# rotationalio/honu

Hardware: AMD Instinct MI355X
Metric: GiB/s + records/s device-resident encode+decode, 1M Large(~300KB) object batch (higher is better)
Workload: dtype u8

## Files before the change

### honu_amd/csrc/api.hip

```cpp
#include <stdio.h>
#include <stdlib.h>
#include <string.h>

#include "kernels.h"

using namespace honu;

struct honu_ctx {
    int device;
    uint64_t max_n;
    LaunchGeom geom;
    void *ws;
    uint64_t *counts;
    uint64_t *offs;
    uint64_t *totals;
    DecodeScratch *scratch;
    uint32_t *reg_inline;
    EncAclPos *enc_acl;
    FusedState dec;
    uint64_t lb_bytes;
    ScanState scan;
    uint32_t spec_off;
    int speculate;
    hipStream_t aux;
    hipEvent_t ev_fork, ev_join;
    int enc_fork;
    bool acl_inplace;
    bool reg_inplace;
    int guard_blocks;
    uint32_t copy_seq;
    int enc_form;
};

static LaunchGeom copy_geom(honu_ctx *ctx) {
    LaunchGeom g = ctx->geom;
    const uint32_t k = __atomic_fetch_add(&ctx->copy_seq, 1u, __ATOMIC_RELAXED) % COPY_TICKET_LINES;
    g.copy_tickets = ctx->geom.copy_tickets + (uint64_t)k * COPY_TICKET_STRIDE;
    return g;
}
static constexpr uint32_t SPEC_BACKOFF_CALLS = 16;
#ifndef SPECULATE_DEFAULT
#define SPECULATE_DEFAULT 2
#endif

static thread_local char g_last_error[256];

static int32_t hip_fail(hipError_t e, const char *what) {
    snprintf(g_last_error, sizeof g_last_error, "%s: %s", what, hipGetErrorString(e));
    return HONU_E_HIP;
}
#define HIPCHK(x)                                  \
    do {                                           \
        hipError_t e_ = (x);                       \
        if (e_ != hipSuccess) return hip_fail(e_, #x); \
    } while (0)

static int32_t arg_fail(const char *what) {
    snprintf(g_last_error, sizeof g_last_error, "invalid argument: %s", what);
    return HONU_E_ARG;
}

static bool aligned(const void *p, uintptr_t a) { return ((uintptr_t)p & (a - 1)) == 0; }

#define FUSED_DECODE_MIN_RECORDS (48ull << 10)

static int fused_blocks(const LaunchGeom &g) {
    const int resident = 2 * g.num_cu;
    return g.lane_blocks > 0 && g.lane_blocks < resident ? g.lane_blocks : resident;
}

template <class T>
static uint64_t carve(T *&p, void *base, uint64_t at, uint64_t count) {
    p = (T *)((uintptr_t)base + at);
    return at + count * sizeof(T);
}

static uint64_t ctx_carve(honu_ctx *c, void *base) {
    const uint64_t n = c->max_n;
    const uint64_t tiles = (n + HONU_WAVE - 1) / HONU_WAVE;
    const uint64_t groups = (tiles / HONU_WAVE + 1) > LB_GROUPS ? tiles / HONU_WAVE + 1 : LB_GROUPS;
    uint64_t at = 0;
    at = carve(c->counts, base, at, 3 * n);
    at = carve(c->offs, base, at, 3 * n);
    at = carve(c->totals, base, at, 4);
    at = carve(c->scratch, base, at, n);
    at = carve(c->reg_inline, base, at, 8 * n);
    at = carve(c->enc_acl, base, at, n);
    at = carve(c->dec.lb, base, at, 1);
    at = carve(c->scan.lb, base, at, 1);
    at = carve(c->dec.status, base, at, 3 * tiles);
    at = carve(c->dec.gstatus, base, at, 3 * groups);
    c->dec.words = 3 * tiles + 3 * groups;
    c->scan.words = scan_status_words(n);
    at = carve(c->scan.status, base, at, c->scan.words);
    return carve(c->geom.copy_tickets, base, at, (uint64_t)COPY_TICKET_LINES * COPY_TICKET_STRIDE);
}

static bool stream_is_restricted(hipStream_t s, int num_cu) {
    int prio = 0;
    if (hipStreamGetPriority(s, &prio) == hipSuccess && prio != 0) return true;
    uint32_t mask[32] = {0};
    const uint32_t words = (uint32_t)((num_cu + 31) / 32);
    if (words > 32 || hipExtStreamGetCUMask(s, words, mask) != hipSuccess) return false;
    bool any = false, all = true;
    for (int i = 0; i < num_cu; i++) {
        const bool on = mask[i / 32] >> (i % 32) & 1u;
        any |= on;
        all &= on;
    }
    return any && !all;
}

static int env_int(const char *name, int dflt) {
#ifdef HONU_AB
    const char *v = getenv(name);
    return v && *v ? atoi(v) : dflt;
#else
    (void)name;
    return dflt;
#endif
}

extern "C" {

uint32_t honu_abi_version(void) { return HONU_ABI_VERSION; }
uint64_t honu_sizeof_meta(void) { return sizeof(honu_meta); }
uint64_t honu_sizeof_acl(void) { return sizeof(honu_acl); }
uint64_t honu_sizeof_collection(void) { return sizeof(honu_collection); }
uint64_t honu_sizeof_index(void) { return sizeof(honu_index); }
uint64_t honu_sizeof_record_info(void) { return sizeof(honu_record_info); }
uint64_t honu_sizeof_seek(void) { return sizeof(honu_seek); }
uint64_t honu_sizeof_list_row(void) { return sizeof(honu_list_row); }
uint64_t honu_sizeof_next(void) { return sizeof(honu_next); }
const char *honu_last_error(void) { return g_last_error; }

const char *honu_status_string(int32_t st) {
    switch (st) {
    case HONU_OK: return "ok";
    case HONU_ERR_BAD_VERSION: return "object is malformed: cannot decode specified version";
    case HONU_ERR_MALFORMED: return "object is malformed: cannot parse data or metadata";
    case HONU_ERR_EOF: return "EOF";
    case HONU_ERR_UNEXPECTED_EOF: return "unexpected EOF";
    case HONU_ERR_NO_LENGTH: return "field not written with length value";
    case HONU_ERR_PARSE_BOOLEAN: return "could not parse boolean value";
    case HONU_ERR_PARSE_VARINT: return "could not parse varint";
    case HONU_ERR_PANIC: return "input on which the Go reference panics";
    case HONU_ERR_CAPACITY: return "output capacity exceeded";
    case HONU_ERR_INPUT: return "input span or list outside its arena";
    case HONU_UNPARSED: return "metadata not decoded (headers only)";
    case HONU_E_ARG: return "invalid argument";
    case HONU_E_WORKSPACE: return "batch larger than the context's reserved records";
    case HONU_E_HIP: return "HIP runtime error";
    case HONU_E_NO_DEVICE: return "no gfx950 device";
    default: return "unknown status";
    }
}

honu_ctx *honu_ctx_create(int device, uint64_t max_records, int32_t *err) {
    int32_t dummy;
    if (!err) err = &dummy;
    *err = HONU_OK;
    int count = 0;
    if (hipGetDeviceCount(&count) != hipSuccess || device < 0 || device >= count) {
        snprintf(g_last_error, sizeof g_last_error, "no HIP device %d (count %d)", device, count);
        *err = HONU_E_NO_DEVICE;
        return nullptr;
    }
    hipDeviceProp_t prop;
    if (hipGetDeviceProperties(&prop, device) != hipSuccess ||
        strncmp(prop.gcnArchName, "gfx950", 6) != 0) {
        snprintf(g_last_error, sizeof g_last_error, "device %d is %s, this build targets gfx950",
                 device, prop.gcnArchName);
        *err = HONU_E_NO_DEVICE;
        return nullptr;
    }
    if (hipSetDevice(device) != hipSuccess) {
        *err = HONU_E_HIP;
        return nullptr;
    }
    honu_ctx *c = (honu_ctx *)calloc(1, sizeof(honu_ctx));
    if (!c) {
        *err = HONU_E_HIP;
        return nullptr;
    }
    auto fail = [&](int32_t e, const char *what) -> honu_ctx * {
        if (what) snprintf(g_last_error, sizeof g_last_error, "%s", what);
        if (c->ev_join) (void)hipEventDestroy(c->ev_join);
        if (c->ev_fork) (void)hipEventDestroy(c->ev_fork);
        if (c->aux) (void)hipStreamDestroy(c->aux);
        if (c->dec.spec_seen) (void)hipHostFree(c->dec.spec_seen);
        if (c->ws) (void)hipFree(c->ws);
        free(c);
        *err = e;
        return nullptr;
    };
    c->device = device;
    c->max_n = max_records ? max_records : 1;
    c->geom.num_cu = prop.multiProcessorCount;
    c->geom.per_record_blocks = env_int("HONU_RECORD_BLOCKS", prop.multiProcessorCount * 8);
    c->geom.lane_blocks = env_int("HONU_LANE_BLOCKS", 0);
    c->geom.copy_blocks = env_int("HONU_COPY_BLOCKS", prop.multiProcessorCount * 2);
    c->geom.record_variant = env_int("HONU_RECORD_VARIANT", 0);
    if (c->geom.record_variant != 5 && c->geom.record_variant != 6)
        c->geom.record_variant = 0;
    c->acl_inplace = env_int("HONU_ACL_INPLACE", 1) != 0;
    c->reg_inplace = env_int("HONU_REGIONS_INPLACE", 1) != 0;
    c->guard_blocks = env_int("HONU_GUARD_BLOCKS", 0);
    if (c->guard_blocks < 0) c->guard_blocks = 0;
    const uint64_t end = ctx_carve(c, nullptr), bytes = end + 256;
    if (hipMalloc(&c->ws, bytes) != hipSuccess) {
        c->ws = nullptr;
        char msg[96];
        snprintf(msg, sizeof msg, "hipMalloc(%llu) failed", (unsigned long long)bytes);
        return fail(HONU_E_HIP, msg);
    }
    if (hipHostMalloc((void **)&c->dec.spec_seen, 2 * sizeof(uint32_t),
                      hipHostMallocMapped | hipHostMallocCoherent) != hipSuccess) {
        c->dec.spec_seen = nullptr;
        return fail(HONU_E_HIP, "hipHostMalloc(spec_seen) failed");
    }
    c->dec.spec_seen[0] = 0;
    c->dec.spec_seen[1] = 0;
    c->speculate = SPECULATE_DEFAULT;
    c->enc_fork = env_int("HONU_ENCODE_FORK", 2);
    if (c->enc_fork < 0 || c->enc_fork > 2) c->enc_fork = 2;
    if (hipStreamCreateWithFlags(&c->aux, hipStreamNonBlocking) != hipSuccess) {
        c->aux = nullptr;
        return fail(HONU_E_HIP, "stream creation failed");
    }
    if (hipEventCreateWithFlags(&c->ev_fork, hipEventDisableTiming) != hipSuccess) {
        c->ev_fork = nullptr;
        return fail(HONU_E_HIP, "event creation failed");
    }
    if (hipEventCreateWithFlags(&c->ev_join, hipEventDisableTiming) != hipSuccess) {
        c->ev_join = nullptr;
        return fail(HONU_E_HIP, "event creation failed");
    }
    ctx_carve(c, c->ws);
    c->lb_bytes = (uint64_t)((uint8_t *)c->ws + end - (uint8_t *)c->dec.lb);
    c->geom.copy_steal = 1;
    c->scan.max_blocks = 4 * prop.multiProcessorCount;
    hipStream_t s = nullptr;
    bool ok = hipStreamCreateWithFlags(&s, hipStreamNonBlocking) == hipSuccess;
    ok = ok && hipMemsetAsync(c->dec.lb, 0, c->lb_bytes, s) == hipSuccess;
    ok = ok && hipStreamSynchronize(s) == hipSuccess;
    if (s) (void)hipStreamDestroy(s);
    if (!ok) return fail(HONU_E_HIP, "look-back state initialisation failed");
    return c;
}

int32_t honu_ctx_reset(honu_ctx *ctx, void *stream) {
    if (!ctx) return arg_fail("ctx");
    HIPCHK(hipSetDevice(ctx->device));
    HIPCHK(hipMemsetAsync(ctx->dec.lb, 0, ctx->lb_bytes, (hipStream_t)stream));
    HIPCHK(hipStreamSynchronize((hipStream_t)stream));
    return HONU_OK;
}

void honu_ctx_destroy(honu_ctx *ctx) {
    if (!ctx) return;
    (void)hipSetDevice(ctx->device);
    (void)hipStreamSynchronize(ctx->aux);
    (void)hipEventDestroy(ctx->ev_fork);
    (void)hipEventDestroy(ctx->ev_join);
    (void)hipStreamDestroy(ctx->aux);
    (void)hipFree(ctx->ws);
    (void)hipHostFree(ctx->dec.spec_seen);
    free(ctx);
}

uint64_t honu_ctx_max_records(const honu_ctx *ctx) { return ctx ? ctx->max_n : 0; }

int32_t honu_ctx_set_param(honu_ctx *ctx, const char *name, int64_t value) {
    if (!ctx || !name) return arg_fail("ctx/name");
    if (!strcmp(name, "copy_blocks") && value > 0) ctx->geom.copy_blocks = (int)value;
    else if (!strcmp(name, "record_blocks") && value > 0) ctx->geom.per_record_blocks = (int)value;
    else if (!strcmp(name, "lane_blocks") && value >= 0) ctx->geom.lane_blocks = (int)value;
    else if (!strcmp(name, "speculate") && value >= 0 && value <= 2) ctx->speculate = (int)value;
    else if (!strcmp(name, "encode_fork") && value >= 0 && value <= 2) ctx->enc_fork = (int)value;
    else if (!strcmp(name, "acl_inplace") && (value == 0 || value == 1)) ctx->acl_inplace = value != 0;
    else if (!strcmp(name, "regions_inplace") && (value == 0 || value == 1)) ctx->reg_inplace = value != 0;
    else if (!strcmp(name, "guard_blocks") && value >= 0 && value <= 65536) ctx->guard_blocks = (int)value;
    else if (!strcmp(name, "speculate_backoff") && value >= 0 && value <= (int64_t)SPEC_BACKOFF_CALLS) {
        __atomic_store_n(ctx->dec.spec_seen, 0u, __ATOMIC_RELAXED);
        ctx->spec_off = (uint32_t)value;
    }
    else if (!strcmp(name, "copy_steal") && (value == 0 || value == 1)) ctx->geom.copy_steal = (int)value;
    else if (!strcmp(name, "copy_variant") || !strcmp(name, "encode_variant") || !strcmp(name, "inline_recovery")) {
        if (value != 0) return arg_fail(name);
    }
    else if (!strcmp(name, "record_variant") &&
             (value == 0 || value == 5 || value == 6))
        ctx->geom.record_variant = (int)value;
    else if (!strcmp(name, "seek_variant") && value >= 0 && value <= 2) ctx->geom.seek_variant = (int)value;
    else return arg_fail(name);
    return HONU_OK;
}

int32_t honu_ctx_get_param(const honu_ctx *ctx, const char *name, int64_t *value) {
    if (!ctx || !name || !value) return arg_fail("ctx/name/value");
    if (!strcmp(name, "copy_blocks")) *value = ctx->geom.copy_blocks;
    else if (!strcmp(name, "record_blocks")) *value = ctx->geom.per_record_blocks;
    else if (!strcmp(name, "lane_blocks")) *value = ctx->geom.lane_blocks;
    else if (!strcmp(name, "speculate")) *value = ctx->speculate;
    else if (!strcmp(name, "encode_fork")) *value = ctx->enc_fork;
    else if (!strcmp(name, "acl_inplace")) *value = ctx->acl_inplace ? 1 : 0;
    else if (!strcmp(name, "regions_inplace")) *value = ctx->reg_inplace ? 1 : 0;
    else if (!strcmp(name, "guard_blocks")) *value = ctx->guard_blocks;
    else if (!strcmp(name, "recoveries"))
        *value = __atomic_load_n(ctx->dec.spec_seen + 1, __ATOMIC_RELAXED);
    else if (!strcmp(name, "speculate_backoff"))
        *value = __atomic_load_n(ctx->dec.spec_seen, __ATOMIC_RELAXED) ? SPEC_BACKOFF_CALLS : ctx->spec_off;
    else if (!strcmp(name, "copy_steal")) *value = ctx->geom.copy_steal;
    else if (!strcmp(name, "copy_variant") || !strcmp(name, "encode_variant") || !strcmp(name, "inline_recovery"))
        *value = 0;
    else if (!strcmp(name, "record_variant")) *value = ctx->geom.record_variant;
    else if (!strcmp(name, "walk_flag_checks")) *value = decode_walk_flag_checks();
    else if (!strcmp(name, "sort_tile")) *value = sort_tile();
    else if (!strcmp(name, "seek_variant")) *value = ctx->geom.seek_variant;
    else if (!strcmp(name, "seek_fence")) *value = seek_fence();
    else if (!strcmp(name, "seek_auto_probes")) *value = (int64_t)seek_auto_probes();
    else if (!strcmp(name, "seek_auto_keys")) *value = (int64_t)seek_auto_keys();
    else if (!strcmp(name, "merge_tile")) *value = merge_tile();
    else if (!strcmp(name, "delete_tile")) *value = delete_tile();
    else if (!strcmp(name, "list_tile")) *value = list_tile();
    else if (!strcmp(name, "list_stage")) *value = list_stage();
    else if (!strcmp(name, "filter_tile")) *value = filter_tile();
    else if (!strcmp(name, "compare_tile")) *value = compare_tile();
    else if (!strcmp(name, "compare_stage")) *value = compare_stage();
    else if (!strcmp(name, "reclaim_tile")) *value = reclaim_tile();
    else return arg_fail(name);
    return HONU_OK;
}

int32_t honu_encode_sizes(honu_ctx *ctx, const honu_meta *d_meta, uint64_t var_len,
                          const honu_acl *d_acl, uint64_t acl_len, const uint32_t *d_regions,
                          uint64_t regions_len, const uint64_t *d_payload_off, uint64_t n,
                          uint64_t *d_sizes, int32_t *d_status, void *stream) {
    if (!ctx) return arg_fail("ctx");
    if (n && (!d_meta || !d_payload_off || !d_sizes)) return arg_fail("null pointer");
    if (!aligned(d_meta, 16)) return arg_fail("rows must be 16-byte aligned");
    if (!aligned(d_acl, 4) || !aligned(d_regions, 4)) return arg_fail("tables must be 4-byte aligned");
    HIPCHK(hipSetDevice(ctx->device));
    HIPCHK(launch_encode_sizes_grp(d_meta, var_len, d_acl, acl_len, d_regions, regions_len,
                                   d_payload_off, n, d_sizes, d_status, ctx->geom.lane_blocks,
                                   (hipStream_t)stream));
    return HONU_OK;
}

int32_t honu_exclusive_scan(honu_ctx *ctx, const uint64_t *d_in, uint64_t n, uint64_t *d_out,
                            void *stream) {
    if (!ctx) return arg_fail("ctx");
    if (n > ctx->max_n) return HONU_E_WORKSPACE;
    HIPCHK(hipSetDevice(ctx->device));
    HIPCHK(launch_scan(d_in, n, 1, d_out, d_out + n, ctx->scan, (hipStream_t)stream));
    return HONU_OK;
}

static int32_t encode_records(honu_ctx *ctx, const honu_meta *d_meta, const uint8_t *d_var,
                              const honu_acl *d_acl, const uint32_t *d_regions, const uint8_t *units,
                              const uint64_t *d_payload_off, uint64_t n, uint8_t *d_out,
                              uint64_t out_cap, const uint64_t *d_out_off, int32_t *d_status,
                              void *stream) {
    if (!ctx) return arg_fail("ctx");
    if (n && (!d_meta || !d_payload_off || !d_out || !d_out_off || !d_status))
        return arg_fail("null pointer");
    if (!aligned(d_out, 16) || !aligned(d_meta, 16))
        return arg_fail("records arena and rows must be 16-byte aligned");
    if (!aligned(d_acl, 4) || !aligned(d_regions, 4)) return arg_fail("tables must be 4-byte aligned");
    HIPCHK(hipSetDevice(ctx->device));
    if (n > ctx->max_n) return HONU_E_WORKSPACE;
    ctx->enc_form = units ? 2 : 1;
    hipStream_t s = (hipStream_t)stream;
    const bool fork = ctx->enc_fork == 1 ||
                      (ctx->enc_fork == 2 && ctx->geom.lane_blocks > 0 && n &&
                       !stream_is_restricted(s, ctx->geom.num_cu));
    if (fork && n) {
        HIPCHK(hipEventRecord(ctx->ev_fork, s));
        HIPCHK(hipStreamWaitEvent(ctx->aux, ctx->ev_fork, 0));
        HIPCHK(launch_encode_acl_grp_self(d_meta, d_acl, d_payload_off, n, d_out, out_cap, d_out_off, d_status,
                                          ctx->geom.lane_blocks, ctx->aux));
        HIPCHK(hipEventRecord(ctx->ev_join, ctx->aux));
        HIPCHK(launch_encode_meta_lane(d_meta, d_var, d_acl, d_regions, d_payload_off, n, d_out,
                                       out_cap, d_out_off, d_status, ctx->enc_acl,
                                       ctx->geom.lane_blocks, ctx->geom.num_cu, units, s));
        HIPCHK(hipStreamWaitEvent(s, ctx->ev_join, 0));
        return HONU_OK;
    }
    HIPCHK(launch_encode_meta_lane(d_meta, d_var, d_acl, d_regions, d_payload_off, n, d_out,
                                   out_cap, d_out_off, d_status, ctx->enc_acl,
                                   ctx->geom.lane_blocks, ctx->geom.num_cu, units, s));
    HIPCHK(launch_encode_acl_grp(d_meta, d_acl, n, d_out, d_status, ctx->enc_acl,
                                 ctx->geom.lane_blocks, s));
    return HONU_OK;
}

int32_t honu_encode_records(honu_ctx *ctx, const honu_meta *d_meta, const uint8_t *d_var,
                            const honu_acl *d_acl, const uint32_t *d_regions,
                            const uint64_t *d_payload_off, uint64_t n, uint8_t *d_out,
                            uint64_t out_cap, const uint64_t *d_out_off, int32_t *d_status,
                            void *stream) {
    return encode_records(ctx, d_meta, d_var, d_acl, d_regions, nullptr, d_payload_off, n, d_out, out_cap,
                          d_out_off, d_status, stream);
}

int32_t honu_encode_records_units(honu_ctx *ctx, const honu_meta *d_meta, const uint8_t *d_var,
                                  const honu_acl *d_acl, const uint32_t *d_regions,
                                  const uint8_t *d_payload, const uint64_t *d_payload_off, uint64_t n,
                                  uint8_t *d_out, uint64_t out_cap, const uint64_t *d_out_off,
                                  int32_t *d_status, void *stream) {
    if (n && !d_payload) return arg_fail("null pointer");
    return encode_records(ctx, d_meta, d_var, d_acl, d_regions, d_payload, d_payload_off, n, d_out, out_cap,
                          d_out_off, d_status, stream);
}

static int32_t encode_payloads(honu_ctx *ctx, const uint8_t *d_payload, const uint64_t *d_payload_off,
                               uint64_t n, uint8_t *d_out, uint64_t out_cap, const uint64_t *d_out_off,
                               const int32_t *d_status, bool units, void *stream) {
    if (!ctx) return arg_fail("ctx");
    if (n && (!d_payload_off || !d_out || !d_out_off || !d_status)) return arg_fail("null pointer");
    if (!aligned(d_out, 16)) return arg_fail("records arena must be 16-byte aligned");
    if (ctx->enc_form && ctx->enc_form != (units ? 2 : 1))
        return arg_fail(units ? "honu_encode_payloads_units after honu_encode_records (mixed forms)"
                              : "honu_encode_payloads after honu_encode_records_units (mixed forms)");
    HIPCHK(hipSetDevice(ctx->device));
    HIPCHK(launch_encode_copy(copy_geom(ctx), d_payload, d_payload_off, n, d_out, out_cap, d_out_off,
                              d_status, units, (hipStream_t)stream));
    return HONU_OK;
}

int32_t honu_encode_payloads(honu_ctx *ctx, const uint8_t *d_payload, const uint64_t *d_payload_off,
                             uint64_t n, uint8_t *d_out, uint64_t out_cap, const uint64_t *d_out_off,
                             const int32_t *d_status, void *stream) {
    return encode_payloads(ctx, d_payload, d_payload_off, n, d_out, out_cap, d_out_off, d_status, false, stream);
}

int32_t honu_encode_payloads_units(honu_ctx *ctx, const uint8_t *d_payload, const uint64_t *d_payload_off,
                                   uint64_t n, uint8_t *d_out, uint64_t out_cap, const uint64_t *d_out_off,
                                   const int32_t *d_status, void *stream) {
    return encode_payloads(ctx, d_payload, d_payload_off, n, d_out, out_cap, d_out_off, d_status, true, stream);
}

int32_t honu_encode(honu_ctx *ctx, const honu_meta *d_meta, const uint8_t *d_var, uint64_t var_len,
                    const honu_acl *d_acl, uint64_t acl_len, const uint32_t *d_regions,
                    uint64_t regions_len, const uint8_t *d_payload, const uint64_t *d_payload_off,
                    uint64_t n, uint8_t *d_out, uint64_t out_cap, const uint64_t *d_out_off,
                    int32_t *d_status, void *stream) {
    (void)var_len;
    (void)acl_len;
    (void)regions_len;
    if (!d_payload) {
        int32_t st = honu_encode_records(ctx, d_meta, d_var, d_acl, d_regions, d_payload_off, n, d_out,
                                         out_cap, d_out_off, d_status, stream);
        if (st) return st;
        return honu_encode_payloads(ctx, d_payload, d_payload_off, n, d_out, out_cap, d_out_off, d_status,
                                    stream);
    }
    int32_t st = honu_encode_records_units(ctx, d_meta, d_var, d_acl, d_regions, d_payload, d_payload_off, n,
                                           d_out, out_cap, d_out_off, d_status, stream);
    if (st) return st;
    return honu_encode_payloads_units(ctx, d_payload, d_payload_off, n, d_out, out_cap, d_out_off,
                                      d_status, stream);
}

int32_t honu_marshal_batch(honu_ctx *ctx, const honu_meta *d_meta, const uint8_t *d_var,
                           uint64_t var_len, const honu_acl *d_acl, uint64_t acl_len,
// ... 644 lines not shown
```

### honu_amd/csrc/copy.hip

```cpp
#include "kernels.h"

namespace honu {

struct EncodeSegments {
    const uint8_t *payload;
    const uint64_t *payload_off;
    uint8_t *out;
    uint64_t out_cap;
    const uint64_t *out_off;
    const int32_t *status;

    HONU_DEV uint64_t start(uint64_t i) const { return payload_off[i]; }
    HONU_DEV uint64_t lo() const { return payload_off[0]; }
    bool units;
    HONU_DEV bool get(uint64_t i, uint64_t &len, const uint8_t *&src, uint8_t *&dst, uint64_t &skip) const {
        const int32_t st = status[i];
        const uint64_t o0 = out_off[i], o1 = out_off[i + 1];
        const uint64_t s = payload_off[i];
        len = payload_off[i + 1] - s;
        src = payload + s;
        dst = out + o0 + 1 + uvarint_len(len);
        skip = 0;
        if (units) {
            const uint64_t a0 = (uint64_t)dst, a1 = a0 + len;
            const uint64_t h_end = ((a0 + PAYLOAD_UNIT - 1) & ~(PAYLOAD_UNIT - 1)) < a1
                                       ? ((a0 + PAYLOAD_UNIT - 1) & ~(PAYLOAD_UNIT - 1)) : a1;
            const uint64_t t_beg = (a1 & ~(PAYLOAD_UNIT - 1)) > h_end ? (a1 & ~(PAYLOAD_UNIT - 1)) : h_end;
            skip = h_end - a0;
            len = t_beg - h_end;
            src += skip;
            dst += skip;
        }
        return st == HONU_OK && o1 <= out_cap && len != 0;
    }
};

struct DecodeSegments {
    const uint8_t *rec;
    const honu_record_info *info;
    const DecodeScratch *scratch;
    const uint64_t *offs;
    uint8_t *data;

    HONU_DEV uint64_t start(uint64_t i) const { return offs[3 * i + 2]; }
    HONU_DEV uint64_t lo() const { return 0; }
    uint64_t n_;
    HONU_DEV bool get(uint64_t i, uint64_t &len, const uint8_t *&src, uint8_t *&dst, uint64_t &skip) const {
        skip = 0;
        const int32_t st = info[i].data_status;
        len = info[i].data_len;
        src = rec + scratch[i].data_src;
        dst = data + offs[3 * i + 2];
        return st == HONU_OK && len != 0;
    }
};

struct SpanSegments {
    const uint8_t *rec;
    const honu_record_info *info;
    const DecodeScratch *scratch;
    const uint64_t *offs;
    uint8_t *data;

    HONU_DEV uint64_t start(uint64_t i) const { return offs[i]; }
    HONU_DEV uint64_t lo() const { return 0; }
    HONU_DEV bool get(uint64_t i, uint64_t &len, const uint8_t *&src, uint8_t *&dst, uint64_t &skip) const {
        skip = 0;
        const int32_t st = info[i].data_status;
        len = info[i].data_len;
        src = rec + scratch[i].data_src;
        dst = data + offs[i];
        return st == HONU_OK && len != 0;
    }
};

struct FetchSegments {
    const honu_list_row *rows;
    const uint8_t *rec;
    const uint64_t *rec_off;
    const uint64_t *val_off;
    uint8_t *values;
    uint64_t val_cap;

    HONU_DEV uint64_t start(uint64_t g) const { return val_off[g]; }
    HONU_DEV uint64_t lo() const { return 0; }
    HONU_DEV bool get(uint64_t g, uint64_t &len, const uint8_t *&src, uint8_t *&dst, uint64_t &skip) const {
        skip = 0;
        const uint64_t o0 = val_off[g], o1 = val_off[g + 1];
        const uint32_t r = rows[g].record;
        len = o1 - o0;
        const bool ok = len != 0 && o1 <= val_cap;
        src = rec + (ok ? rec_off[r] : 0);
        dst = values + o0;
        return ok;
    }
};

struct ReclaimSegments {
    const uint32_t *source;
    const uint8_t *rec;
    const uint64_t *rec_off;
    const uint64_t *val_off;
    uint8_t *values;
    uint64_t val_cap;

    HONU_DEV uint64_t start(uint64_t j) const { return val_off[j]; }
    HONU_DEV uint64_t lo() const { return 0; }
    HONU_DEV bool get(uint64_t j, uint64_t &len, const uint8_t *&src, uint8_t *&dst, uint64_t &skip) const {
        skip = 0;
        const uint64_t o0 = val_off[j], o1 = val_off[j + 1];
        const uint32_t r = source[j];
        len = o1 - o0;
        const bool ok = len != 0 && o1 <= val_cap;
        src = rec + (ok ? rec_off[r] : 0);
        dst = values + o0;
        return ok;
    }
};

#define SMALL_SEG_WAVES_FACTOR 4
#ifndef COPY_FEW_WAVES_MIN
#define COPY_FEW_WAVES_MIN (64u << 10)
#endif
constexpr int COPY_UNROLL = 4;

template <class Seg>
HONU_DEV void copy_short_run(const Seg &seg, uint64_t i0, uint64_t i1, uint64_t short_max) {
    uint64_t len_nx = 0, skip = 0;
    const uint8_t *src_nx = nullptr;
    uint8_t *dst_nx = nullptr;
    bool ok_nx = i0 < i1 && seg.get(i0, len_nx, src_nx, dst_nx, skip);
    for (uint64_t i = i0; i < i1; i++) {
        const uint64_t len = len_nx;
        const uint8_t *src = src_nx;
        uint8_t *dst = dst_nx;
        const bool ok = ok_nx;
        if (i + 1 < i1) ok_nx = seg.get(i + 1, len_nx, src_nx, dst_nx, skip);
        if (ok && len < short_max) wave_copy<COPY_UNROLL>(dst, src, len);
    }
}

template <class Seg>
HONU_DEV void copy_range(const Seg &seg, uint64_t n, uint64_t lo, uint64_t hi, bool skip_short,
                         uint64_t short_max) {
    if (lo >= hi) return;
    uint64_t a = 0, b = n;
    while (b - a > 1) {
        const uint64_t mid = (a + b) >> 1;
        if (seg.start(mid) <= lo) a = mid;
        else b = mid;
    }
    uint64_t s_nx = seg.start(a), len_nx = 0, skip_nx = 0;
    const uint8_t *src_nx = nullptr;
    uint8_t *dst_nx = nullptr;
    bool ok_nx = seg.get(a, len_nx, src_nx, dst_nx, skip_nx);
    for (uint64_t i = a; i < n; i++) {
        const uint64_t s0 = s_nx, len = len_nx, s = s0 + skip_nx;
        const uint8_t *src = src_nx;
        uint8_t *dst = dst_nx;
        const bool ok = ok_nx;
        if (s0 >= hi) break;
        if (i + 1 < n) {
            s_nx = seg.start(i + 1);
            ok_nx = seg.get(i + 1, len_nx, src_nx, dst_nx, skip_nx);
        }
        if (!ok) continue;
        if (skip_short && len < short_max) continue;
        const uint64_t x = s > lo ? s : lo;
        const uint64_t e = s + len;
        const uint64_t y = e < hi ? e : hi;
        if (x < y)
            wave_copy<COPY_UNROLL>(dst + (x - s), src + (x - s), y - x);
    }
}

#define COPY_STEAL_MIN (16u << 10)
#define COPY_STEAL 8u
template <class Seg>
__global__ __launch_bounds__(HONU_BLOCK) void k_copy_segments(Seg seg, uint64_t n,
                                                               const uint64_t *__restrict__ total_p,
                                                               uint64_t short_max, uint32_t *tickets,
                                                               uint32_t steal) {
    uint64_t W = (uint64_t)gridDim.x * HONU_WAVES_PER_BLOCK;
    const uint64_t w = (uint64_t)blockIdx.x * HONU_WAVES_PER_BLOCK + wave_in_block();
    const uint64_t base = seg.lo();
    const uint64_t total = *total_p - base;
    const bool few = n && total / n >= COPY_FEW_WAVES_MIN;
    if (few) {
        const uint64_t Wall = W;
        W /= SMALL_SEG_WAVES_FACTOR;
        if (w >= W) {
            const uint64_t v = w - W, V = Wall - W;
            copy_short_run(seg, n * v / V, n * (v + 1) / V, short_max);
            return;
        }
    }
    if (w >= W) return;
    auto range = [&](uint64_t v, uint64_t &lo, uint64_t &hi) {
        lo = base + ((total * v / W) & ~15ull);
        hi = (v + 1 == W) ? base + total : base + ((total * (v + 1) / W) & ~15ull);
    };
    uint64_t lo, hi;
    range(w, lo, hi);
    if (tickets && n && total / n >= COPY_STEAL_MIN) {
        auto cut = [&](uint64_t l, uint64_t h) {
            return h - ((((h - l) * steal) >> 6) & ~15ull);
        };
        copy_range(seg, n, lo, cut(lo, hi), few, short_max);
        for (;;) {
            uint32_t t = 0;
            if (__lane_id() == 0) t = atomicAdd(&tickets[0], 1u);
            t = __shfl(t, 0);
            if (t >= W) break;
            uint64_t l, h;
            range(t, l, h);
            copy_range(seg, n, cut(l, h), h, few, short_max);
        }
        if (__lane_id() == 0 && atomicAdd(&tickets[1], 1u) == (uint32_t)W - 1) {
            atomicExch(&tickets[0], 0u);
            atomicExch(&tickets[1], 0u);
        }
        return;
    }
    copy_range(seg, n, lo, hi, few, short_max);
}

template <class Seg>
static hipError_t launch_copy(const LaunchGeom &g, const Seg &seg, uint64_t n,
                              const uint64_t *total, uint32_t *tickets, hipStream_t s) {
    const dim3 grid(g.copy_blocks * SMALL_SEG_WAVES_FACTOR), block(HONU_BLOCK);
    hipLaunchKernelGGL((k_copy_segments<Seg>), grid, block, 0, s, seg, n, total,
                       (uint64_t)COPY_FEW_WAVES_MIN, g.copy_steal ? tickets : nullptr, COPY_STEAL);
    return hipGetLastError();
}

hipError_t launch_encode_copy(const LaunchGeom &g, const uint8_t *payload,
                              const uint64_t *payload_off, uint64_t n, uint8_t *out,
                              uint64_t out_cap, const uint64_t *out_off, const int32_t *status,
                              bool units, hipStream_t s) {
    if (n == 0) return hipSuccess;
    EncodeSegments seg{payload, payload_off, out, out_cap, out_off, status, units};
    return launch_copy(g, seg, n, payload_off + n, g.copy_tickets, s);
}

hipError_t launch_span_copy(const LaunchGeom &g, const uint8_t *rec, uint64_t n,
                            const honu_record_info *info, const DecodeScratch *scratch,
                            const uint64_t *offs, uint8_t *data, hipStream_t s) {
    if (n == 0) return hipSuccess;
    SpanSegments seg{rec, info, scratch, offs, data};
    return launch_copy(g, seg, n, offs + n, g.copy_tickets, s);
}

hipError_t launch_decode_copy(const LaunchGeom &g, const uint8_t *rec, uint64_t n,
                              const honu_record_info *info, const DecodeScratch *scratch,
                              const uint64_t *offs, const uint64_t *totals, uint8_t *data,
                              hipStream_t s) {
    if (n == 0) return hipSuccess;
    DecodeSegments seg{rec, info, scratch, offs, data, n};
    return launch_copy(g, seg, n, totals + 2, g.copy_tickets, s);
}

hipError_t launch_fetch_copy(const LaunchGeom &g, const honu_list_row *rows, uint64_t n, const uint8_t *rec,
                             const uint64_t *rec_off, const uint64_t *val_off, uint8_t *values,
                             uint64_t val_cap, hipStream_t s) {
    if (n == 0) return hipSuccess;
    FetchSegments seg{rows, rec, rec_off, val_off, values, val_cap};
    return launch_copy(g, seg, n, val_off + n, g.copy_tickets, s);
}

hipError_t launch_reclaim_copy(const LaunchGeom &g, const uint32_t *source, uint64_t n, const uint8_t *rec,
                               const uint64_t *rec_off, const uint64_t *val_off, uint8_t *values,
                               uint64_t val_cap, hipStream_t s) {
    if (n == 0) return hipSuccess;
    ReclaimSegments seg{source, rec, rec_off, val_off, values, val_cap};
    return launch_copy(g, seg, n, val_off + n, g.copy_tickets, s);
}

}
```

### honu_amd/csrc/kernels.h

```cpp
#pragma once

#include "common.h"
#include "lookback.h"

namespace honu {

struct DecodeScratch {
    uint64_t acl_pos;
    uint64_t regions_pos;
    uint64_t data_src;
    uint64_t rec_end;
};

#define GRP_ACL_FAST (1ull << 63)
#define GRP_REG_INLINE (1ull << 62)
#define GRP_ACL_A0_SHIFT 56
#define GRP_ACL_A0(pos) (((pos) >> GRP_ACL_A0_SHIFT) & 15ull)
#define GRP_ACL_TL_SHIFT 53
#define GRP_ACL_TL(pos) (((pos) >> GRP_ACL_TL_SHIFT) & 7ull)
#define GRP_POS_MASK ((1ull << GRP_ACL_TL_SHIFT) - 1)
#define ACL_ALL_PRESENT (1ull << 63)
#define PAYLOAD_UNIT 64ull

HONU_DEV void acl_enc_words(const honu_acl *e, uint32_t d[5]) {
    const uint32_t *w = reinterpret_cast<const uint32_t *>(e);
    const uint32_t e0 = w[0], e1 = w[1], e2 = w[2], e3 = w[3], e4 = w[4];
    d[0] = 1u | (e0 << 8);
    d[1] = (e0 >> 24) | (e1 << 8);
    d[2] = (e1 >> 24) | (e2 << 8);
    d[3] = (e2 >> 24) | (e3 << 8);
    d[4] = (e3 >> 24) | ((e4 & 0xFF) << 8);
}

HONU_DEV u32x4 acl_chunk(const honu_acl *A, uint64_t na, uint64_t P, uint64_t X) {
    const uint64_t j0 = (X - P) / 18;
    uint32_t b[10];
    acl_enc_words(A + j0, b);
    b[5] = b[6] = b[7] = b[8] = b[9] = 0;
    if (j0 + 1 < na) {
        uint32_t d[5];
        acl_enc_words(A + j0 + 1, d);
        b[4] = (b[4] & 0xFFFF) | (d[0] << 16);
        b[5] = (d[0] >> 16) | (d[1] << 16);
        b[6] = (d[1] >> 16) | (d[2] << 16);
        b[7] = (d[2] >> 16) | (d[3] << 16);
        b[8] = (d[3] >> 16) | (d[4] << 16);
    }
    const uint32_t off = (uint32_t)(X - (P + 18 * j0));
    const uint32_t q = off >> 2, sh = off & 3;
    uint32_t o[4];
#pragma unroll
    for (int k = 0; k < 4; k++) {
        uint32_t w0 = b[k], w1 = b[k + 1];
#pragma unroll
        for (int t = 1; t <= 4; t++)
            if ((uint32_t)t == q) {
                w0 = b[t + k];
                w1 = b[t + k + 1];
            }
        o[k] = __builtin_amdgcn_alignbyte(w1, w0, sh);
    }
    return u32x4{o[0], o[1], o[2], o[3]};
}

struct LaunchGeom {
    int num_cu;
    int per_record_blocks;
    int lane_blocks;
    int copy_blocks;
    int record_variant;
    int seek_variant;
    uint32_t *copy_tickets;
    int copy_steal;
};
#define COPY_TICKET_STRIDE 32u
#define COPY_TICKET_LINES 64u

hipError_t launch_encode_copy(const LaunchGeom &g, const uint8_t *payload,
                              const uint64_t *payload_off, uint64_t n, uint8_t *out,
                              uint64_t out_cap, const uint64_t *out_off, const int32_t *status,
                              bool units, hipStream_t s);

hipError_t launch_decode_copy(const LaunchGeom &g, const uint8_t *rec, uint64_t n,
                              const honu_record_info *info, const DecodeScratch *scratch,
                              const uint64_t *offs, const uint64_t *totals, uint8_t *data,
                              hipStream_t s);
hipError_t launch_decode_keys(const LaunchGeom &g, const honu_meta *meta,
                              const honu_record_info *info, uint64_t n, uint8_t *keys,
                              int32_t *key_status, hipStream_t s);

struct EncAclPos {
    uint64_t pos;
    uint64_t acl_off;
    uint64_t acl_count;
    uint64_t carried;
};
#define ENC_ACL_SIZED (1ull << 63)

hipError_t launch_encode_meta_lane(const honu_meta *meta, const uint8_t *var, const honu_acl *acl,
                                   const uint32_t *reg, const uint64_t *payload_off, uint64_t n,
                                   uint8_t *out, uint64_t out_cap, const uint64_t *out_off,
                                   int32_t *status, EncAclPos *acl_out, int max_blocks, int num_cu,
                                   const uint8_t *payload, hipStream_t s);
hipError_t launch_encode_acl_grp(const honu_meta *meta, const honu_acl *acl, uint64_t n,
                                 uint8_t *out, int32_t *status, const EncAclPos *acl_pos,
                                 int max_blocks, hipStream_t s);
hipError_t launch_encode_acl_grp_self(const honu_meta *meta, const honu_acl *acl, const uint64_t *payload_off,
                                      uint64_t n, uint8_t *out, uint64_t out_cap, const uint64_t *out_off,
                                      int32_t *status, int max_blocks, hipStream_t s);

hipError_t launch_encode_sizes_grp(const honu_meta *meta, uint64_t var_len, const honu_acl *acl,
                                   uint64_t acl_len, const uint32_t *reg, uint64_t reg_len,
                                   const uint64_t *payload_off, uint64_t n, uint64_t *sizes,
                                   int32_t *status, int max_blocks, hipStream_t s);
hipError_t launch_decode_fill_grp(const uint8_t *rec, uint64_t n, honu_meta *meta,
                                  honu_record_info *info, const DecodeScratch *scratch,
                                  const uint32_t *reg_inline, const uint64_t *counts,
                                  const uint64_t *offs, honu_acl *acl, uint64_t acl_cap,
                                  uint32_t *reg, uint64_t reg_cap, uint8_t *data,
                                  uint64_t data_cap, int max_blocks, hipStream_t s);

int decode_walk_flag_checks();
struct DecodeOut {
    honu_meta *meta;
    honu_record_info *info;
    honu_acl *acl;
    uint64_t acl_cap;
    uint32_t *reg;
    uint64_t reg_cap;
    uint64_t data_cap;
    int materialize;
    DecodeScratch *scratch;
    uint64_t *offs;
    uint64_t *totals;
    bool reg_inplace;
};
struct FusedState {
    LbState *lb;
    uint64_t *status, *gstatus;
    uint64_t words;
    uint32_t *spec_seen;
};
struct FusedOpts {
    int max_blocks;
    int guard_blocks;
    bool speculate;
    bool acl_inplace;
};
hipError_t launch_decode_fused(const uint8_t *rec, const uint64_t *rec_off, uint64_t n,
                               const DecodeOut &O, const FusedState &F, const FusedOpts &opt, hipStream_t s);

hipError_t launch_decode_parse_win(const uint8_t *rec, const uint64_t *rec_off, uint64_t n,
                                   honu_meta *meta, honu_record_info *info,
                                   DecodeScratch *scratch, uint32_t *reg_inline, uint64_t *counts,
                                   int max_blocks, bool inplace, bool reg_inplace, hipStream_t s);

hipError_t launch_system_sizes(const honu_collection *rows, uint64_t var_len, const honu_acl *acl,
                               uint64_t acl_len, const uint32_t *reg, uint64_t reg_len,
                               const honu_index *idx, uint64_t idx_len, uint64_t n,
                               uint64_t *sizes, int32_t *status, hipStream_t s);
hipError_t launch_system_encode(const honu_collection *rows, const uint8_t *var,
                                const honu_acl *acl, const uint32_t *reg, const honu_index *idx,
                                uint64_t n, uint8_t *out, uint64_t out_cap,
                                const uint64_t *out_off, int32_t *status, hipStream_t s);
hipError_t launch_system_parse(const uint8_t *rec, const uint64_t *rec_off, uint64_t n,
                               bool headless, honu_collection *rows, int32_t *status,
                               DecodeScratch *scratch, uint64_t *counts, hipStream_t s);
hipError_t launch_system_fill(const uint8_t *rec, uint64_t n, honu_collection *rows,
                              int32_t *status, const DecodeScratch *scratch,
                              const uint64_t *counts, const uint64_t *offs, honu_acl *acl,
                              uint64_t acl_cap, uint32_t *reg, uint64_t reg_cap, honu_index *idx,
                              uint64_t idx_cap, hipStream_t s);

hipError_t launch_decode_headers(const uint8_t *rec, const uint64_t *rec_off, uint64_t n,
                                 honu_record_info *info, hipStream_t s);
hipError_t launch_decode_spans(const uint8_t *rec, const uint64_t *rec_off, uint64_t n,
                               honu_record_info *info, DecodeScratch *scratch, uint64_t *counts,
                               hipStream_t s);
hipError_t launch_decode_data_place(uint64_t n, honu_record_info *info, const uint64_t *offs,
                                    uint64_t data_cap, hipStream_t s);
hipError_t launch_span_copy(const LaunchGeom &g, const uint8_t *rec, uint64_t n,
                            const honu_record_info *info, const DecodeScratch *scratch,
                            const uint64_t *offs, uint8_t *data, hipStream_t s);

struct ScanState {
    LbState *lb;
    uint64_t *status;
    uint64_t words;
    int max_blocks;
};
uint64_t scan_status_words(uint64_t n);
hipError_t launch_scan(const uint64_t *in, uint64_t n, int K, uint64_t *out, uint64_t *totals,
                       const ScanState &S, hipStream_t s);

inline uint64_t up256(uint64_t x) { return (x + 255) & ~255ull; }

struct SortWork {
    uint32_t *plan;
    u32x4 *key[2];
    uint32_t *idx[2];
    uint64_t *col;
    uint64_t *table;
};
uint32_t sort_tile();
uint64_t sort_workspace_bytes(uint64_t n);
SortWork sort_carve(void *work, uint64_t n);
hipError_t launch_sort_keys(const uint8_t *keys, const int32_t *status, uint64_t n, uint32_t *order,
                            uint8_t *sorted, uint64_t *valid, void *work, const ScanState &S,
                            uint64_t scan_rows, hipStream_t s);
hipError_t launch_key_objects(const uint8_t *keys, const uint32_t *order, const uint64_t *valid, uint64_t n,
                              uint64_t *obj_off, uint32_t *latest, uint64_t *objects, void *work,
                              const ScanState &S, hipStream_t s);

uint32_t seek_fence();
uint64_t seek_auto_probes();
uint64_t seek_auto_keys();
hipError_t launch_key_seek(int variant, int num_cu, const uint8_t *sorted, const uint64_t *valid, uint64_t n,
                           const uint8_t *probes, const int32_t *pstatus, uint32_t probe_len, uint64_t m,
                           const uint32_t *order, const honu_record_info *info, honu_seek *out, hipStream_t s);

uint32_t merge_tile();
hipError_t launch_key_merge(const uint8_t *sa, const uint32_t *oa, const uint64_t *valid_a, uint64_t na,
                            const uint8_t *sb, const uint32_t *ob, const uint64_t *valid_b, uint64_t nb,
                            uint32_t b_base, uint8_t *out, uint32_t *order, uint64_t *valid_out, hipStream_t s);

uint32_t delete_tile();
// ... 76 lines not shown
```

Measured before the change: 1351.

## Split copy-kernel stolen tails into geometrically shrinking pieces with a larger share

The copy kernel's work-stealing tail changes from one fixed share per wave to a configurable share split into up to four geometrically shrinking pieces, handed out through the atomic ticket counter. The share doubles when not in few-records mode. Segment lookup now uses a wave-parallel search instead of a serial binary search, and optional stage-timing stamps are added behind a compile flag. The goal is better load balance at the end of the large copy, at the cost of more atomic tickets and per-ticket index arithmetic.

```diff
diff --git a/honu_amd/csrc/api.hip b/honu_amd/csrc/api.hip
--- a/honu_amd/csrc/api.hip
+++ b/honu_amd/csrc/api.hip
@@ -38,6 +38,9 @@
     g.copy_tickets = ctx->geom.copy_tickets + (uint64_t)k * COPY_TICKET_STRIDE;
     return g;
 }
+static constexpr int COPY_TAIL_SHARE_DEFAULT = 8, COPY_TAIL_PIECES_DEFAULT = 4;
+static constexpr int64_t COPY_BLOCKS_MAX = 1 << 24;
+static_assert(16ull * COPY_BLOCKS_MAX * (COPY_PIECES_MAX + 1) < (1ull << 32), "ticket counter");
 static constexpr uint32_t SPEC_BACKOFF_CALLS = 16;
 #ifndef SPECULATE_DEFAULT
 #define SPECULATE_DEFAULT 2
@@ -200,6 +203,7 @@
     c->geom.per_record_blocks = env_int("HONU_RECORD_BLOCKS", prop.multiProcessorCount * 8);
     c->geom.lane_blocks = env_int("HONU_LANE_BLOCKS", 0);
     c->geom.copy_blocks = env_int("HONU_COPY_BLOCKS", prop.multiProcessorCount * 2);
+    if (c->geom.copy_blocks < 1 || c->geom.copy_blocks > COPY_BLOCKS_MAX) c->geom.copy_blocks = prop.multiProcessorCount * 2;
     c->geom.record_variant = env_int("HONU_RECORD_VARIANT", 0);
     if (c->geom.record_variant != 5 && c->geom.record_variant != 6)
         c->geom.record_variant = 0;
@@ -239,6 +243,8 @@
     ctx_carve(c, c->ws);
     c->lb_bytes = (uint64_t)((uint8_t *)c->ws + end - (uint8_t *)c->dec.lb);
     c->geom.copy_steal = 1;
+    c->geom.copy_tail_pieces = COPY_TAIL_PIECES_DEFAULT;
+    c->geom.copy_tail_share = COPY_TAIL_SHARE_DEFAULT;
     c->scan.max_blocks = 4 * prop.multiProcessorCount;
     hipStream_t s = nullptr;
     bool ok = hipStreamCreateWithFlags(&s, hipStreamNonBlocking) == hipSuccess;
@@ -273,7 +279,7 @@
 
 int32_t honu_ctx_set_param(honu_ctx *ctx, const char *name, int64_t value) {
     if (!ctx || !name) return arg_fail("ctx/name");
-    if (!strcmp(name, "copy_blocks") && value > 0) ctx->geom.copy_blocks = (int)value;
+    if (!strcmp(name, "copy_blocks") && value > 0 && value <= COPY_BLOCKS_MAX) ctx->geom.copy_blocks = (int)value;
     else if (!strcmp(name, "record_blocks") && value > 0) ctx->geom.per_record_blocks = (int)value;
     else if (!strcmp(name, "lane_blocks") && value >= 0) ctx->geom.lane_blocks = (int)value;
     else if (!strcmp(name, "speculate") && value >= 0 && value <= 2) ctx->speculate = (int)value;
@@ -286,6 +292,9 @@
         ctx->spec_off = (uint32_t)value;
     }
     else if (!strcmp(name, "copy_steal") && (value == 0 || value == 1)) ctx->geom.copy_steal = (int)value;
+    else if (!strcmp(name, "copy_tail_pieces") && value >= 1 && value <= (int64_t)COPY_PIECES_MAX)
+        ctx->geom.copy_tail_pieces = (int)value;
+    else if (!strcmp(name, "copy_tail_share") && value >= 1 && value <= 32) ctx->geom.copy_tail_share = (int)value;
     else if (!strcmp(name, "copy_variant") || !strcmp(name, "encode_variant") || !strcmp(name, "inline_recovery")) {
         if (value != 0) return arg_fail(name);
     }
@@ -312,6 +321,8 @@
     else if (!strcmp(name, "speculate_backoff"))
         *value = __atomic_load_n(ctx->dec.spec_seen, __ATOMIC_RELAXED) ? SPEC_BACKOFF_CALLS : ctx->spec_off;
     else if (!strcmp(name, "copy_steal")) *value = ctx->geom.copy_steal;
+    else if (!strcmp(name, "copy_tail_pieces")) *value = ctx->geom.copy_tail_pieces;
+    else if (!strcmp(name, "copy_tail_share")) *value = ctx->geom.copy_tail_share;
     else if (!strcmp(name, "copy_variant") || !strcmp(name, "encode_variant") || !strcmp(name, "inline_recovery"))
         *value = 0;
     else if (!strcmp(name, "record_variant")) *value = ctx->geom.record_variant;
diff --git a/honu_amd/csrc/copy.hip b/honu_amd/csrc/copy.hip
--- a/honu_amd/csrc/copy.hip
+++ b/honu_amd/csrc/copy.hip
@@ -1,4 +1,5 @@
 #include "kernels.h"
+#include "keycol.h"
 
 namespace honu {
 
@@ -141,15 +142,39 @@
 }
 
 template <class Seg>
-HONU_DEV void copy_range(const Seg &seg, uint64_t n, uint64_t lo, uint64_t hi, bool skip_short,
-                         uint64_t short_max) {
-    if (lo >= hi) return;
+HONU_DEV uint64_t first_segment(const Seg &seg, uint64_t n, uint64_t lo) {
+    if (n <= 0xFFFFFFFFull)
+        return wave_bound(1u, (uint32_t)n, [&](uint32_t m) { return seg.start(m) <= lo; }) - 1;
     uint64_t a = 0, b = n;
     while (b - a > 1) {
         const uint64_t mid = (a + b) >> 1;
         if (seg.start(mid) <= lo) a = mid;
         else b = mid;
     }
+    return a;
+}
+
+#ifdef HONU_STAGE_TIMING
+constexpr uint32_t COPY_STAMP_WAVES = 1u << 14, COPY_STAMP_SLOTS = 16, COPY_STAMP_TAKES = 11;
+static __device__ uint64_t g_copy_stamp[COPY_STAMP_WAVES][COPY_STAMP_SLOTS];
+#define COPY_STAMP(w_, k_)                                                                            \
+    do {                                                                                              \
+        if (__lane_id() == 0 && (w_) < COPY_STAMP_WAVES) g_copy_stamp[w_][k_] = wall_clock64();       \
+    } while (0)
+#define COPY_STAMP_VALUE(w_, k_, v_)                                                                  \
+    do {                                                                                              \
+        if (__lane_id() == 0 && (w_) < COPY_STAMP_WAVES) g_copy_stamp[w_][k_] = (v_);                 \
+    } while (0)
+#else
+#define COPY_STAMP(w_, k_) do {} while (0)
+#endif
+
+template <class Seg>
+HONU_DEV void copy_range(const Seg &seg, uint64_t n, uint64_t lo, uint64_t hi, bool skip_short,
+                         uint64_t short_max, uint64_t stamp_w = ~0ull) {
+    if (lo >= hi) return;
+    const uint64_t a = first_segment(seg, n, lo);
+    COPY_STAMP(stamp_w, 1);
     uint64_t s_nx = seg.start(a), len_nx = 0, skip_nx = 0;
     const uint8_t *src_nx = nullptr;
     uint8_t *dst_nx = nullptr;
@@ -175,16 +200,16 @@
 }
 
 #define COPY_STEAL_MIN (16u << 10)
-#define COPY_STEAL 8u
 template <class Seg>
 __global__ __launch_bounds__(HONU_BLOCK) void k_copy_segments(Seg seg, uint64_t n,
                                                                const uint64_t *__restrict__ total_p,
                                                                uint64_t short_max, uint32_t *tickets,
-                                                               uint32_t steal) {
+                                                               uint32_t share_few, uint32_t pieces) {
     uint64_t W = (uint64_t)gridDim.x * HONU_WAVES_PER_BLOCK;
     const uint64_t w = (uint64_t)blockIdx.x * HONU_WAVES_PER_BLOCK + wave_in_block();
     const uint64_t base = seg.lo();
     const uint64_t total = *total_p - base;
+    COPY_STAMP(w, 0);
     const bool few = n && total / n >= COPY_FEW_WAVES_MIN;
     if (few) {
         const uint64_t Wall = W;
@@ -192,37 +217,45 @@
         if (w >= W) {
             const uint64_t v = w - W, V = Wall - W;
             copy_short_run(seg, n * v / V, n * (v + 1) / V, short_max);
+            COPY_STAMP(w, 3);
             return;
         }
     }
     if (w >= W) return;
-    auto range = [&](uint64_t v, uint64_t &lo, uint64_t &hi) {
-        lo = base + ((total * v / W) & ~15ull);
-        hi = (v + 1 == W) ? base + total : base + ((total * (v + 1) / W) & ~15ull);
-    };
     uint64_t lo, hi;
-    range(w, lo, hi);
+    split_range(total, W, w, &lo, &hi);
     if (tickets && n && total / n >= COPY_STEAL_MIN) {
-        auto cut = [&](uint64_t l, uint64_t h) {
-            return h - ((((h - l) * steal) >> 6) & ~15ull);
-        };
-        copy_range(seg, n, lo, cut(lo, hi), few, short_max);
+        const uint32_t share = few || pieces == 1 ? share_few : 2 * share_few;
+        auto take = [&]() { return __lane_id() == 0 ? atomicAdd(&tickets[0], 1u) : 0u; };
+        copy_range(seg, n, base + lo, base + split_cut(lo, hi, share, pieces), few, short_max, w);
+        COPY_STAMP(w, 2);
+        const uint64_t T = W * split_pieces_used(total, W, share, pieces, COPY_PIECE_MIN);
+#ifdef HONU_STAGE_TIMING
+        uint32_t taken = 0;
+#endif
         for (;;) {
-            uint32_t t = 0;
-            if (__lane_id() == 0) t = atomicAdd(&tickets[0], 1u);
-            t = __shfl(t, 0);
-            if (t >= W) break;
-            uint64_t l, h;
-            range(t, l, h);
-            copy_range(seg, n, cut(l, h), h, few, short_max);
-        }
+            const uint32_t t = __shfl(take(), 0);
+            if (t >= T) break;
+#ifdef HONU_STAGE_TIMING
+            if (taken < COPY_STAMP_TAKES) COPY_STAMP(w, 5 + taken);
+            taken++;
+#endif
+            uint64_t a, b;
+            split_ticket(total, W, share, pieces, COPY_PIECE_MIN, t, &a, &b);
+            copy_range(seg, n, base + a, base + b, few, short_max);
+        }
+#ifdef HONU_STAGE_TIMING
+        COPY_STAMP_VALUE(w, 4, (uint64_t)taken);
+#endif
+        COPY_STAMP(w, 3);
         if (__lane_id() == 0 && atomicAdd(&tickets[1], 1u) == (uint32_t)W - 1) {
             atomicExch(&tickets[0], 0u);
             atomicExch(&tickets[1], 0u);
         }
         return;
     }
-    copy_range(seg, n, lo, hi, few, short_max);
+    copy_range(seg, n, base + lo, base + hi, few, short_max, w);
+    COPY_STAMP(w, 3);
 }
 
 template <class Seg>
@@ -230,7 +263,8 @@
                               const uint64_t *total, uint32_t *tickets, hipStream_t s) {
     const dim3 grid(g.copy_blocks * SMALL_SEG_WAVES_FACTOR), block(HONU_BLOCK);
     hipLaunchKernelGGL((k_copy_segments<Seg>), grid, block, 0, s, seg, n, total,
-                       (uint64_t)COPY_FEW_WAVES_MIN, g.copy_steal ? tickets : nullptr, COPY_STEAL);
+                       (uint64_t)COPY_FEW_WAVES_MIN, g.copy_steal ? tickets : nullptr,
+                       (uint32_t)g.copy_tail_share, (uint32_t)g.copy_tail_pieces);
     return hipGetLastError();
 }
 
@@ -277,3 +311,17 @@
 }
 
 }
+
+#ifdef HONU_STAGE_TIMING
+extern "C" int32_t honu_debug_copy_stamps(void *host, uint64_t waves, int32_t reset) {
+    using namespace honu;
+    if (waves > COPY_STAMP_WAVES) return -1;
+    if (reset) {
+        void *p = nullptr;
+        if (hipGetSymbolAddress(&p, HIP_SYMBOL(g_copy_stamp)) != hipSuccess) return -1;
+        return hipMemset(p, 0, sizeof(uint64_t) * COPY_STAMP_WAVES * COPY_STAMP_SLOTS) == hipSuccess ? 0 : -1;
+    }
+    return hipMemcpyFromSymbol(host, HIP_SYMBOL(g_copy_stamp), waves * COPY_STAMP_SLOTS * sizeof(uint64_t)) ==
+                   hipSuccess ? 0 : -1;
+}
+#endif
diff --git a/honu_amd/csrc/copy_split.h b/honu_amd/csrc/copy_split.h
--- /dev/null
+++ b/honu_amd/csrc/copy_split.h
@@ -0,0 +1,56 @@
+#pragma once
+
+#include <stdint.h>
+
+#ifndef HONU_SPLIT_FN
+#define HONU_SPLIT_FN static inline
+#endif
+
+#define COPY_PIECE_MIN (64ull << 10)
+#define COPY_PIECES_MAX 8u
+
+HONU_SPLIT_FN void split_range(uint64_t total, uint64_t W, uint64_t v, uint64_t *lo, uint64_t *hi) {
+    *lo = (total * v / W) & ~15ull;
+    *hi = v + 1 == W ? total : (total * (v + 1) / W) & ~15ull;
+}
+
+HONU_SPLIT_FN uint64_t split_cut(uint64_t lo, uint64_t hi, uint32_t share, uint32_t pieces) {
+    const uint64_t c = hi - ((((hi - lo) * share) >> 6) & ~15ull);
+    return pieces > 1 ? c & ~15ull : c;
+}
+
+HONU_SPLIT_FN void split_piece(uint64_t cut, uint64_t hi, uint32_t pieces, uint64_t piece_min, uint32_t k,
+                               uint64_t *a, uint64_t *b) {
+    uint64_t at = cut;
+    for (uint32_t j = 0;; j++) {
+        const uint64_t left = hi - at;
+        const uint64_t rest = (left >> 1) & ~15ull;
+        const uint64_t end = (j + 1 == pieces || rest < piece_min) ? hi : (hi - rest) & ~15ull;
+        if (j == k) {
+            *a = at;
+            *b = end;
+            return;
+        }
+        at = end;
+    }
+}
+
+HONU_SPLIT_FN uint32_t split_pieces_used(uint64_t total, uint64_t W, uint32_t share, uint32_t pieces,
+                                         uint64_t piece_min) {
+    uint64_t left = (((total / W + 32) * share) >> 6) + 16;
+    uint32_t k = 1;
+    while (k < pieces) {
+        const uint64_t rest = (left >> 1) & ~15ull;
+        if (rest < piece_min) break;
+        left = rest + 15;
+        k++;
+    }
+    return k;
+}
+
+HONU_SPLIT_FN void split_ticket(uint64_t total, uint64_t W, uint32_t share, uint32_t pieces, uint64_t piece_min,
+                                uint64_t t, uint64_t *a, uint64_t *b) {
+    uint64_t lo, hi;
+    split_range(total, W, t % W, &lo, &hi);
+    split_piece(split_cut(lo, hi, share, pieces), hi, pieces, piece_min, (uint32_t)(t / W), a, b);
+}
diff --git a/honu_amd/csrc/kernels.h b/honu_amd/csrc/kernels.h
--- a/honu_amd/csrc/kernels.h
+++ b/honu_amd/csrc/kernels.h
@@ -2,6 +2,8 @@
 
 #include "common.h"
 #include "lookback.h"
+#define HONU_SPLIT_FN HONU_HD
+#include "copy_split.h"
 
 namespace honu {
 
@@ -72,6 +74,8 @@
     int seek_variant;
     uint32_t *copy_tickets;
     int copy_steal;
+    int copy_tail_pieces;
+    int copy_tail_share;
 };
 #define COPY_TICKET_STRIDE 32u
 #define COPY_TICKET_LINES 64u
```

New measurement: 1308. 0.968x the previous value.
